# huawei-noah/Speech-Backbones

Measured on NVIDIA H100. Metric: mel-frames/sec at N=50 reverse-diffusion steps, higher is better.
Workload: dtype f32

## Files before the change

include/sbk.h:

```cpp
#ifndef SBK_H_
#define SBK_H_

#include <stddef.h>
#include <stdint.h>

#ifdef __cplusplus
extern "C" {
#endif

typedef struct sbk_handle sbk_handle;

enum { SBK_OK = 0, SBK_ERR_ARG = 1, SBK_ERR_CUDA = 2, SBK_ERR_STATE = 3, SBK_ERR_UNSUPPORTED = 4 };

enum { SBK_PREC_FP32 = 0,
       SBK_PREC_TF32 = 1,
       SBK_PREC_BF16 = 2,
       SBK_PREC_FP32X3 = 3 };

enum { SBK_MODEL_GRADTTS = 0, SBK_MODEL_DIFFVC = 1 };

typedef struct sbk_config {
    int32_t model;
    int32_t n_feats;
    int32_t dim;
// ... 9 lines not shown
    int32_t use_ref_t;
} sbk_config;

int sbk_create(const sbk_config* cfg, sbk_handle** out);
void sbk_destroy(sbk_handle* h);

int sbk_set_weight(sbk_handle* h, const char* ref_name, const void* data, const int64_t* shape, int ndim);
int sbk_pack(sbk_handle* h);
int sbk_num_weights(const sbk_handle* h);
const char* sbk_weight_name(const sbk_handle* h, int i);

size_t sbk_workspace_bytes(const sbk_handle* h, int B, int T);
size_t sbk_workspace_bytes_n(const sbk_handle* h, int B, int T, int n_timesteps);

int sbk_estimator(sbk_handle* h, const float* x, const float* mask, const float* mu, const float* t,
                  const float* spk, float* out, int B, int T, void* stream);

int sbk_reverse_diffusion(sbk_handle* h, const float* z, const float* mask, const float* mu, const float* spk,
                          const float* noise, float* out, int B, int T, int n_timesteps, int stoc, void* stream);

int sbk_vc_estimator(sbk_handle* h, const float* x, const float* mask, const float* mean, const float* cond,
                     const float* t, float* out, int B, int T, void* stream);

int sbk_vc_reverse_diffusion(sbk_handle* h, const float* z, const float* mask, const float* mean, const float* cond,
                             const float* noise, float* out, int B, int T, int n_timesteps, int mode, void* stream);

int sbk_vc_conditioning(sbk_handle* h, const float* ref, const float* ref_mask, const float* mean_ref, const float* c,
                        float* cond_out, int B, int Tr, int n_timesteps, void* stream);
int sbk_vc_cond_debug_num(const sbk_handle* h);
const char* sbk_vc_cond_debug_name(const sbk_handle* h, int i);
int sbk_vc_cond_debug_op_layout(const sbk_handle* h, const char* name);
int sbk_vc_cond_debug_read(sbk_handle* h, const char* name, void* dst, int64_t* numel);

int sbk_reverse_steps(sbk_handle* h, float* xt, const float* mask, const float* mu, const float* spk,
                      const float* noise, int B, int T, int n_timesteps, int step_begin, int step_end,
                      int stoc, void* stream);

int sbk_reverse_diffusion_host(sbk_handle* h, const float* z, const float* mask, const float* mu, const float* spk,
                               const float* noise, float* out, int B, int T, int n_timesteps, int stoc);

int sbk_prior_expand(const float* mu_x, const float* w_ceil, const float* x_mask, const int64_t* y_lengths,
                     const float* noise_tf, float temperature, int B, int F, int Tx, int Ty,
                     float* mu_y, float* z, float* y_mask, float* attn, void* stream);

int64_t sbk_last_launch_count(const sbk_handle* h);
int sbk_last_host_launches(const sbk_handle* h);

int sbk_profile_ops(sbk_handle* h, float* ms, double* flops, double* bytes, int cap, int* n_ops);

int sbk_debug_read(sbk_handle* h, const char* name, float* dst, int64_t* numel);
int sbk_debug_capture(sbk_handle* h, int on);
int sbk_debug_layout(const sbk_handle* h);
int sbk_debug_op_layout(const sbk_handle* h, const char* name);
int sbk_debug_num(const sbk_handle* h);
const char* sbk_debug_name(const sbk_handle* h, int i);

typedef struct sbk_vocoder sbk_vocoder;
typedef struct sbk_vocoder_config {
    int32_t device;
    int32_t num_mels;
    int32_t upsample_initial_channel;
    int32_t n_ups;
    int32_t upsample_rates[4];
    int32_t upsample_kernel_sizes[4];
    int32_t n_kernels;
    int32_t resblock_kernel_sizes[3];
    int32_t resblock_dilations[3][3];
} sbk_vocoder_config;
int sbk_vocoder_create(const sbk_vocoder_config* cfg, sbk_vocoder** out);
typedef struct sbk_vocoder_config_ex {
    int32_t device;
    int32_t num_mels;
    int32_t upsample_initial_channel;
    int32_t n_ups;
    int32_t upsample_rates[4];
    int32_t upsample_kernel_sizes[4];
    int32_t n_kernels;
    int32_t resblock_kernel_sizes[3];
    int32_t resblock_dilations[3][3];
    int32_t resblock;
} sbk_vocoder_config_ex;
int sbk_vocoder_create_ex(const sbk_vocoder_config_ex* cfg, sbk_vocoder** out);
void sbk_vocoder_destroy(sbk_vocoder* v);
int sbk_vocoder_num_weights(const sbk_vocoder* v);
const char* sbk_vocoder_weight_name(const sbk_vocoder* v, int i);
int sbk_vocoder_set_weight(sbk_vocoder* v, const char* name, const void* data, const int64_t* shape, int ndim);
int sbk_vocoder_pack(sbk_vocoder* v);
int sbk_vocoder_set_precision(sbk_vocoder* v, int32_t precision);
size_t sbk_vocoder_workspace_bytes(const sbk_vocoder* v, int B, int T);
int sbk_vocoder_forward(sbk_vocoder* v, const float* mel, float* wav, int B, int T, void* stream);
int64_t sbk_vocoder_last_launch_count(const sbk_vocoder* v);
int sbk_vocoder_debug_capture(sbk_vocoder* v, int on);
int sbk_vocoder_debug_num(const sbk_vocoder* v);
const char* sbk_vocoder_debug_name(const sbk_vocoder* v, int i);
int sbk_vocoder_debug_read(sbk_vocoder* v, const char* name, float* dst, int64_t* numel);
int sbk_vocoder_debug_op_layout(const sbk_vocoder* v, const char* name);

typedef struct sbk_textenc sbk_textenc;
typedef struct sbk_textenc_config {
    int32_t device;
    int32_t n_vocab, n_feats, n_channels, filter_channels, filter_channels_dp, n_heads, n_layers, kernel_size, window_size;
    int32_t n_spks, spk_emb_dim;
    int32_t kind;
} sbk_textenc_config;
int sbk_textenc_create(const sbk_textenc_config* cfg, sbk_textenc** out);
void sbk_textenc_destroy(sbk_textenc* e);
// ... 34 lines not shown
```

speech-backbones_b200/csrc/sbk_api.cu:

```cuda
#include "sbk_host.h"

#include <math.h>
#include <stdarg.h>
#include <stdio.h>
#include <stdlib.h>
#include <string.h>

#include <algorithm>
#include <map>
#include <string>
#include <vector>

using namespace sbk;

static thread_local char g_err[1024] = "";
int sbk::fail(int code, const char* fmt, ...) {
    va_list ap;
    va_start(ap, fmt);
    vsnprintf(g_err, sizeof(g_err), fmt, ap);
    va_end(ap);
    return code;
}

namespace {
// ... 1194 lines not shown
        vp.out = cond_out + (size_t)i * B * dc; vp.B = B; vp.dc = dc; vp.use_ref = cf.use_ref_t ? 1 : 0;
        n += launch_vc_cond(vp, s);
    }
    if (const cudaError_t e = h->vc_snaps.finish()) return fail(SBK_ERR_CUDA, "sbk_vc_conditioning: debug capture failed: %s", cudaGetErrorString(e));
    CU(cudaGetLastError());
    h->last_launches = n;
    return SBK_OK;
}

extern "C" int sbk_vc_cond_debug_num(const sbk_handle* h) { return h ? (int)h->vc_snaps.list.size() : 0; }
extern "C" const char* sbk_vc_cond_debug_name(const sbk_handle* h, int i) {
    if (!h || i < 0 || i >= (int)h->vc_snaps.list.size()) return nullptr;
    return h->vc_snaps.list[i].name.c_str();
}
extern "C" int sbk_vc_cond_debug_op_layout(const sbk_handle* h, const char* name) {
    const Snapshots::Snap* sn = h && name ? h->vc_snaps.find(name) : nullptr;
    return sn ? sn->fmt : -1;
}
extern "C" int sbk_vc_cond_debug_read(sbk_handle* h, const char* name, void* dst, int64_t* numel) {
    if (!h || !name) return fail(SBK_ERR_ARG, "sbk_vc_cond_debug_read: null argument");
    return h->vc_snaps.read(name, dst, numel, h->cfg.device, "sbk_vc_cond_debug_read");
}

extern "C" int sbk_prior_expand(const float* mu_x, const float* w_ceil, const float* x_mask, const int64_t* y_lengths,
                                const float* noise_tf, float temperature, int B, int F, int Tx, int Ty,
                                float* mu_y, float* z, float* y_mask, float* attn, void* stream) {
    if (!mu_x || !w_ceil || !x_mask || !y_lengths || !mu_y || !z || !y_mask) return fail(SBK_ERR_ARG, "sbk_prior_expand: null argument");
    if (B <= 0 || F <= 0 || Tx <= 0 || Ty <= 0) return fail(SBK_ERR_ARG, "sbk_prior_expand: bad sizes B=%d F=%d Tx=%d Ty=%d", B, F, Tx, Ty);
    if (Tx > 12000) return fail(SBK_ERR_ARG, "sbk_prior_expand: Tx=%d exceeds the 12000-token shared-memory table", Tx);
    if (noise_tf && !(temperature > 0.f)) return fail(SBK_ERR_ARG, "sbk_prior_expand: temperature must be > 0");
    PriorExpandParams p;
    p.mu_x = mu_x; p.w_ceil = w_ceil; p.x_mask = x_mask; p.y_len = reinterpret_cast<const long long*>(y_lengths);
    p.noise_tf = noise_tf; p.temperature = temperature; p.B = B; p.F = F; p.Tx = Tx; p.Ty = Ty;
    p.mu_y = mu_y; p.z = z; p.y_mask = y_mask; p.attn = attn;
    launch_prior_expand(p, (cudaStream_t)stream);
    CU(cudaGetLastError());
    return SBK_OK;
}

extern "C" int64_t sbk_last_launch_count(const sbk_handle* h) { return h ? h->last_launches : 0; }
extern "C" int sbk_last_host_launches(const sbk_handle* h) { return h ? h->last_host_launches : 0; }

extern "C" int sbk_debug_capture(sbk_handle* h, int on) {
    if (!h) return fail(SBK_ERR_ARG, "sbk_debug_capture: null handle");
    h->capture = h->vc_snaps.on = on != 0;
    return SBK_OK;
}
extern "C" int sbk_debug_layout(const sbk_handle* h) { return (h && h->cfg.precision != SBK_PREC_FP32) ? 1 : 0; }
extern "C" int sbk_debug_op_layout(const sbk_handle* h, const char* name) {
    if (!h || !name) return -1;
    for (auto& op : h->plan.ops) if (op.name == name) return op.dbg_fmt;
    return -1;
}
extern "C" int sbk_debug_num(const sbk_handle* h) { return h ? (int)h->plan.ops.size() : 0; }
extern "C" const char* sbk_debug_name(const sbk_handle* h, int i) {
    if (!h || i < 0 || i >= (int)h->plan.ops.size()) return nullptr;
    return h->plan.ops[i].name.c_str();
}
extern "C" int sbk_debug_read(sbk_handle* h, const char* name, float* dst, int64_t* numel) {
    if (!h || !name) return fail(SBK_ERR_ARG, "sbk_debug_read: null argument");
    for (auto& op : h->plan.ops) {
        if (op.name != name) continue;
        if (numel) *numel = op.dbg_numel;
        if (dst && op.dbg_ptr && op.dbg_numel > 0) {
            CU(cudaDeviceSynchronize());
            const void* src = op.dbg_copy ? (const void*)op.dbg_copy : (const void*)op.dbg_ptr;
            return read_widened(dst, src, op.dbg_numel, op.dbg_fmt);
        }
        return SBK_OK;
    }
    return fail(SBK_ERR_ARG, "sbk_debug_read: no intermediate named '%s'", name);
}
```

speech-backbones_b200/csrc/sbk_attn_x3.cu:

```cuda
#include "sbk_tc.cuh"

#include <type_traits>

namespace sbk {

using namespace tc;

namespace kx3 {
constexpr int PX = 64;
constexpr int KCH = 8;
constexpr int XS = KCH * PX * 16;
constexpr int WS = 2 * KCH * 128 * 16;
constexpr int STAGE = XS + WS;
constexpr int STAGES = 2;
constexpr int OPI = (PX / 4) * 128 * 16;
constexpr int THREADS = 256 + 32;
constexpr int NBARS = 2 * STAGES;
constexpr size_t SMEM = (size_t)STAGES * STAGE + 4 * OPI + 4 * 128 * 4 + NBARS * 8 + 16;
static_assert(SMEM <= 227 * 1024, "shared memory budget");
static_assert(XS <= OPI && STAGES == 2, "fp32x3: the converted x fits a context image; a K stage is the whole ring");
}

template <int MODE>
__global__ void __launch_bounds__(kx3::THREADS, 1) k_attn_kv_wg(const ConvTcParams p) {
    using namespace kx3;
    constexpr bool X3 = MODE == 2;
    constexpr int EPC = MODE == 1 ? 8 : 4;
    constexpr int KMAIN = MODE == 1 ? K_BF16 : K_TF32;
    extern __shared__ __align__(1024) uint8_t smem[];
    uint8_t* sS = smem;
    uint8_t* kp = sS + STAGES * STAGE;
    uint8_t* vt = kp + OPI;
    uint8_t* pc = vt + OPI;
    uint8_t* vc = pc + OPI;
    float* s_mx = reinterpret_cast<float*>(vc + OPI);
    float* s_z = s_mx + 2 * 128;
    uint64_t* bars = reinterpret_cast<uint64_t*>(s_z + 2 * 128);

    const int tid = threadIdx.x, warp = __shfl_sync(0xffffffffu, tid >> 5, 0), lane = tid & 31;
    const int HW = p.H * p.W;
    const int ksteps = p.c0 / (KCH * EPC);
    const int ksteps_t = X3 ? 2 * ksteps : ksteps;
    const int items = (HW + PX - 1) / PX;
    const int total = p.B * items;
    const uint32_t bar0 = smem_u32(bars);
    auto full = [&](int s) { return bar0 + 8u * s; };
    auto empty = [&](int s) { return bar0 + 8u * (STAGES + s); };

    if (tid == 0) {
        for (int s = 0; s < STAGES; ++s) { mbar_init(full(s), 1); mbar_init(empty(s), 8); }
        fence_barrier_init();
    }
    __syncthreads();

    if (warp < 8) {
        const int wg = warp >> 2, wt = tid & 127;
        const int row = tid & 127, half = tid >> 7;
        constexpr uint32_t D_HI = desc_hi(128);
        const uint32_t s0 = smem_u32(sS);
        uint32_t it = 0;
        for (int t = blockIdx.x; t < total; t += gridDim.x) {
            const int b = t / items, mt = t - b * items;
            float acc[64];
            if constexpr (X3) {
                for (int kb = 0; kb < ksteps; ++kb, it += 2) {
                    const int sc = it % STAGES, sm = (it + 1) % STAGES;
                    mbar_wait(full(sc), (it / STAGES) & 1);
                    mbar_wait(full(sm), ((it + 1) / STAGES) & 1);
                    const uint32_t xc = s0 + sc * STAGE, xm = s0 + sm * STAGE;
                    uint8_t* cx = (kb & 1) ? vc : pc;
                    {
                        const float4* src = reinterpret_cast<const float4*>(sS + sm * STAGE);
#pragma unroll
                        for (int i = tid; i < XS / 16; i += 256) {
                            const float4 v = src[i];
                            reinterpret_cast<float4*>(cx)[i] = corr_chunk(v.x, v.y, v.z, v.w);
                        }
                    }
                    fence_proxy_async();
                    asm volatile("bar.sync 1, 256;" ::: "memory");
                    const uint32_t c_lo = desc_lo(smem_u32(cx), PX * 16), x_lo = desc_lo(xm, PX * 16);
                    const uint32_t wc_lo = desc_lo(xc + XS + wg * (KCH * 128 * 16), 128 * 16), wm_lo = desc_lo(xm + XS + wg * (KCH * 128 * 16), 128 * 16);
                    wg_fence();
#pragma unroll
                    for (int kk = 0; kk < KCH / 2; ++kk)
                        wgmma<128, K_F16>(acc, desc_pack(c_lo + (uint32_t)(kk * 2 * PX), D_HI), desc_pack(wc_lo + (uint32_t)(kk * 2 * 128), D_HI),
                                          (kb | kk) != 0 ? 1u : 0u);
#pragma unroll
                    for (int kk = 0; kk < KCH / 2; ++kk)
                        wgmma<128, K_TF32>(acc, desc_pack(x_lo + (uint32_t)(kk * 2 * PX), D_HI), desc_pack(wm_lo + (uint32_t)(kk * 2 * 128), D_HI), 1u);
                    wg_commit();
                    wg_wait<0>();
                    wg_fence_regs(acc);
                    __syncwarp();
                    if (lane == 0) { mbar_arrive(empty(sc)); mbar_arrive(empty(sm)); }
                }
            } else
            for (int ks = 0; ks < ksteps_t; ++ks, ++it) {
                const int s = it % STAGES;
                mbar_wait(full(s), (it / STAGES) & 1);
                const uint32_t xs = s0 + s * STAGE;
                const uint32_t x_lo = desc_lo(xs, PX * 16), w_lo = desc_lo(xs + XS + wg * (KCH * 128 * 16), 128 * 16);
                auto issue = [&](auto kind) {
#pragma unroll
                    for (int kk = 0; kk < KCH / 2; ++kk)
                        wgmma<128, decltype(kind)::value>(acc, desc_pack(x_lo + (uint32_t)(kk * 2 * PX), D_HI),
                                                          desc_pack(w_lo + (uint32_t)(kk * 2 * 128), D_HI), (ks | kk) != 0 ? 1u : 0u);
                };
                wg_fence();
                issue(std::integral_constant<int, KMAIN>{});
                wg_commit();
                wg_wait<0>();
                wg_fence_regs(acc);
                __syncwarp();
                if (lane == 0) mbar_arrive(empty(s));
            }
            {
                uint8_t* img = wg == 0 ? kp : vt;
#pragma unroll
                for (int i = 0; i < 64; ++i) {
                    const int px = frag_row(wt, i), r = frag_col(wt, i);
                    *reinterpret_cast<float*>(img + ((size_t)(px / 4) * 128 + r) * 16 + (px % 4) * 4) = acc[i];
                }
            }
            asm volatile("bar.sync 1, 256;" ::: "memory");
            const int nvalid = min(PX, HW - mt * PX) - half * (PX / 2);
            float kr[PX / 2];
#pragma unroll
            for (int c = 0; c < PX / 8; ++c) {
                const float4 q = *reinterpret_cast<const float4*>(kp + ((size_t)(half * (PX / 8) + c) * 128 + row) * 16);
                kr[4 * c] = q.x; kr[4 * c + 1] = q.y; kr[4 * c + 2] = q.z; kr[4 * c + 3] = q.w;
            }
            float mx = -INFINITY;
#pragma unroll
            for (int i = 0; i < PX / 2; ++i) mx = fmaxf(mx, i < nvalid ? kr[i] : -INFINITY);
            s_mx[half * 128 + row] = mx;
            asm volatile("bar.sync 1, 256;" ::: "memory");
            const float md = fmaxf(s_mx[row], s_mx[128 + row]);
            float z0 = 0.f, z1 = 0.f;
#pragma unroll
            for (int i = 0; i < PX / 2; i += 2) {
                const float e0 = i < nvalid ? (X3 ? expf(kr[i] - md) : __expf(kr[i] - md)) : 0.f;
                const float e1 = i + 1 < nvalid ? (X3 ? expf(kr[i + 1] - md) : __expf(kr[i + 1] - md)) : 0.f;
                z0 += e0; z1 += e1;
                kr[i] = e0; kr[i + 1] = e1;
            }
            s_z[half * 128 + row] = z0 + z1;
#pragma unroll
            for (int c = 0; c < PX / 8; ++c) {
                const size_t o = ((size_t)(half * (PX / 8) + c) * 128 + row) * 16;
                const float e0 = kr[4 * c], e1 = kr[4 * c + 1], e2 = kr[4 * c + 2], e3 = kr[4 * c + 3];
                *reinterpret_cast<float4*>(kp + o) = make_float4(e0, e1, e2, e3);
                if constexpr (X3) {
                    *reinterpret_cast<uint4*>(pc + o) =
                        make_uint4(f16x2_sat(tf32_lo(e0) * 256.f, tf32_lo(e1) * 256.f), f16x2_sat(tf32_lo(e2) * 256.f, tf32_lo(e3) * 256.f),
                                   f16x2_sat(e0 * 0.0625f, e1 * 0.0625f), f16x2_sat(e2 * 0.0625f, e3 * 0.0625f));
                    const float4 v = *reinterpret_cast<const float4*>(vt + o);
                    *reinterpret_cast<uint4*>(vc + o) =
                        make_uint4(f16x2_sat(v.x * 0.00390625f, v.y * 0.00390625f), f16x2_sat(v.z * 0.00390625f, v.w * 0.00390625f),
                                   f16x2_sat(tf32_lo(v.x) * 16.f, tf32_lo(v.y) * 16.f), f16x2_sat(tf32_lo(v.z) * 16.f, tf32_lo(v.w) * 16.f));
                }
            }
            fence_proxy_async();
            asm volatile("bar.sync 1, 256;" ::: "memory");
            float sacc[32];
            {
                const uint32_t p_lo = desc_lo(smem_u32(kp) + 64 * wg * 16, 128 * 16), v_lo = desc_lo(smem_u32(vt) + 64 * wg * 16, 128 * 16);
                const uint32_t pc_lo = desc_lo(smem_u32(pc) + 64 * wg * 16, 128 * 16), vc_lo = desc_lo(smem_u32(vc) + 64 * wg * 16, 128 * 16);
                wg_fence();
                if constexpr (X3) {
#pragma unroll
                    for (int kk = 0; kk < PX / 8; ++kk)
                        wgmma<64, K_F16>(sacc, desc_pack(pc_lo + (uint32_t)(kk * 2 * 128), D_HI), desc_pack(vc_lo + (uint32_t)(kk * 2 * 128), D_HI),
                                         kk != 0 ? 1u : 0u);
                }
#pragma unroll
                for (int kk = 0; kk < PX / 8; ++kk)
                    wgmma<64, K_TF32>(sacc, desc_pack(p_lo + (uint32_t)(kk * 2 * 128), D_HI), desc_pack(v_lo + (uint32_t)(kk * 2 * 128), D_HI),
                                      (X3 || kk != 0) ? 1u : 0u);
                wg_commit();
                wg_wait<0>();
                wg_fence_regs(sacc);
            }
            float* pt0 = p.kv_part + ((long long)b * items + mt) * kHeads * kKvPartFloats;
            if (half == 0) {
                float* pt = pt0 + (row / 32) * kKvPartFloats;
                pt[row % 32] = md;
                pt[32 + row % 32] = s_z[row] + s_z[128 + row];
            }
#pragma unroll
            for (int i = 0; i < 32; ++i) {
                const int dl = frag_row(wt, i), el = frag_col(wt, i);
                if ((dl >> 5) == (el >> 5)) {
                    float* pt = pt0 + (2 * wg + (dl >> 5)) * kKvPartFloats;
                    pt[64 + (dl & 31) * 32 + (el & 31)] = sacc[i];
                }
            }
            asm volatile("bar.sync 1, 256;" ::: "memory");
        }
    } else {
        uint32_t it = 0;
        const int chs = p.c0 / EPC;
        for (int t = blockIdx.x; t < total; t += gridDim.x) {
            const int b = t / items, mt = t - b * items;
            const int m0 = mt * PX, m_hi = m0 + PX < HW ? m0 + PX : HW;
            const int hh0 = m0 / p.W, ww0 = m0 - hh0 * p.W;
            for (int ks = 0; ks < ksteps_t; ++ks, ++it) {
                const int s = it % STAGES;
                const int kb = X3 ? ks >> 1 : ks;
                const bool corr = X3 && (ks & 1) == 0;
                const uint32_t xs = smem_u32(sS) + s * STAGE;
                if (lane == 0) {
                    mbar_wait(empty(s), ((it / STAGES) & 1) ^ 1);
                    mbar_arrive_expect_tx(full(s), corr ? WS : STAGE);
                    bulk_g2s(xs + XS, reinterpret_cast<const uint8_t*>(p.wpk) + (size_t)(X3 ? 2 * kb + (corr ? 1 : 0) : ks) * WS, WS, full(s));
                }
                __syncwarp();
                if (lane < KCH && !corr) {
                    const uint8_t* src = reinterpret_cast<const uint8_t*>(p.in0);
                    const int k = lane, cl = kb * KCH + k;
                    int m = m0, hh = hh0, ww = ww0, qx = 0;
                    while (m < m_hi) {
                        const int n = (p.W - ww) < (m_hi - m) ? (p.W - ww) : (m_hi - m);
                        bulk_g2s(xs + (k * PX + qx) * 16, src + (((long long)(b * p.H + hh) * chs + cl) * p.W + ww) * 16,
                                 (uint32_t)n * 16u, full(s));
                        m += n; qx += n; ++hh; ww = 0;
                    }
                    if (qx < PX) bulk_g2s(xs + (k * PX + qx) * 16, p.zero_page, (uint32_t)(PX - qx) * 16u, full(s));
                }
            }
        }
    }
}

template <int MODE>
static int launch_kv(const ConvTcParams& p, cudaStream_t s) {
    static DevCache cache;
    const int num_sms = cache.get(reinterpret_cast<const void*>(k_attn_kv_wg<MODE>));
    if (num_sms <= 0) return -1;
    if (p.c0 % (kx3::KCH * (MODE == 1 ? 8 : 4)) != 0) return -1;
    const long long total = (long long)p.B * ((p.H * p.W + kx3::PX - 1) / kx3::PX);
    const int grid = (int)(total < num_sms ? total : num_sms);
    k_attn_kv_wg<MODE><<<grid, kx3::THREADS, kx3::SMEM, s>>>(p);
    return 1;
}

int attn_kv_tile_pixels() { return kx3::PX; }
int launch_attn_kv(const ConvTcParams& p, cudaStream_t s) {
    return p.form == FORM_X3 ? launch_kv<2>(p, s) : p.form == FORM_BF16 ? launch_kv<1>(p, s) : launch_kv<0>(p, s);
}

}
```

speech-backbones_b200/csrc/sbk_conv_tc.cu:

```cuda
#include "sbk_tc.cuh"

#include <cuda_fp16.h>
#include <string.h>
#include <type_traits>

namespace sbk {

namespace tc {

constexpr int TPX = 128;
constexpr int NCONS = 256;
constexpr int NTHREADS = NCONS + 128;
constexpr int NCONV = 96;
constexpr int PROD_REGS = 40, CONS_REGS = 232;
static_assert(128 * PROD_REGS + NCONS * CONS_REGS <= 65536, "register file");

template <int GEOM, int R = 1> struct Geo;
template <int R> struct Geo<G_C3, R> {
    static_assert(R == 1 || R == 2, "3x3 tiles are 1 or 2 rows");
    static constexpr int ROWS = R, HR = R + 2, PXP = TPX + 2, TAPS = 9, KCH = 2, NACC = R;
};
template <> struct Geo<G_PW> { static constexpr int ROWS = 1, HR = 1, PXP = TPX, TAPS = 1, KCH = 8, NACC = 1; };
template <> struct Geo<G_DOWN> { static constexpr int ROWS = 1, HR = 3, PXP = 2 * (TPX + 1), TAPS = 9, KCH = 2, NACC = 1; };
template <> struct Geo<G_UP> { static constexpr int ROWS = 1, HR = 3, PXP = TPX + 2, TAPS = 16, KCH = 2, NACC = 4; };
// ... 734 lines not shown
        case tc_key(G_C7, T, 64):                   return launch_tc<G_C7, T, 64>(p, s);
        case tc_key(G_C7, X, 64):                   return launch_tc<G_C7, X, 64>(p, s);
        default:                                    return -1;
    }
}

static uint32_t f32_to_tf32_rna(float x) {
    uint32_t u; memcpy(&u, &x, 4);
    if ((u & 0x7F800000u) != 0x7F800000u) u += 0x1000u;
    return u & 0xFFFFE000u;
}
static uint16_t f32_to_f16_rn(float x) {
    if (x > 65504.f) x = 65504.f;
    if (x < -65504.f) x = -65504.f;
    const __half h = __float2half_rn(x);
    uint16_t u; memcpy(&u, &h, 2);
    return u;
}
static uint16_t f32_to_bf16_rn(float x) {
    uint32_t u; memcpy(&u, &x, 4);
    if ((u & 0x7FFFFFFFu) > 0x7F800000u) return (uint16_t)((u >> 16) | 0x40);
    u += 0x7FFFu + ((u >> 16) & 1u);
    return (uint16_t)(u >> 16);
}
static void wimg_put(uint8_t* img, const ConvTcWImg& g, int co, int ks, int tap, int ch, int e, float w) {
    const size_t i = conv_tc_wimg_index(g, co, ks, tap, ch, e);
    if (g.form == FORM_BF16) {
        reinterpret_cast<uint16_t*>(img)[i] = f32_to_bf16_rn(w);
        return;
    }
    const uint32_t uh = f32_to_tf32_rna(w);
    reinterpret_cast<uint32_t*>(img)[i] = uh;
    if (g.form == FORM_X3) {
        float fh; memcpy(&fh, &uh, 4);
        uint16_t* cc = reinterpret_cast<uint16_t*>(img) + 2 * conv_tc_wimg_index(g, co, ks, tap, ch, 0, 1);
        cc[e] = f32_to_f16_rn(w);
        cc[4 + e] = f32_to_f16_rn((w - fh) * 4096.f);
    }
}

size_t conv_tc_pack_image(const float* w, int cout, int cin, int geom, int form, int nt, uint8_t* dst) {
    const ConvTcWImg g = conv_tc_wimg(geom, form, nt, cin);
    const int taps = conv_tc_taps(geom), rows = conv_tc_stage_rows(geom), epc = form_epc(form), cps = g.kch * epc;
    if (dst)
        for (int co = 0; co < cout / nt * nt; ++co) for (int ks = 0; ks < g.ksteps; ++ks) for (int tap = 0; tap < g.taps; ++tap)
            for (int ch = 0; ch < g.kch; ++ch) for (int e = 0; e < epc; ++e) {
                const int ci = ks / rows * cps + ch * epc + e;
                wimg_put(dst, g, co, ks, tap, ch, e, w[((size_t)co * cin + ci) * taps + ks % rows * g.taps + tap]);
            }
    return conv_tc_wimg_bytes(g, cout);
}

size_t attn_kv_pack_image(const float* q, int C, int form, uint8_t* dst) {
    ConvTcWImg g = conv_tc_wimg(G_PW, form, 128, C);
    g.taps = 2;
    const int epc = form_epc(form), cps = g.kch * epc;
    if (dst)
        for (int row = 0; row < 128; ++row) for (int ks = 0; ks < g.ksteps; ++ks) for (int kv = 0; kv < 2; ++kv)
            for (int ch = 0; ch < g.kch; ++ch) for (int e = 0; e < epc; ++e)
                wimg_put(dst, g, row, ks, kv, ch, e, q[(size_t)(128 + kv * 128 + row) * C + ks * cps + ch * epc + e]);
    return conv_tc_wimg_bytes(g, 128);
}

}
```

speech-backbones_b200/csrc/sbk_internal.h:

```cpp
#pragma once
#include <cuda_runtime.h>
#include <stdint.h>

namespace sbk {

constexpr int kGroups = 8;
constexpr int kHeads = 4;
constexpr int kDimHead = 32;
constexpr int kAttnHidden = 128;
constexpr int kKvPartFloats = 32 + 32 + 32 * 32;

enum Geom { G_PW = 0, G_C3 = 1, G_DOWN = 2, G_UP = 3, G_C1K3 = 4, G_C1K7 = 5, G_C1K11 = 6, G_C7 = 7, G_C1K5 = 8,
            G_C1K3W = 9, G_C1K5W = 10, G_C1K7W = 11, G_C1K11W = 12 };
__host__ __device__ constexpr bool geom_c1_wide(int g) { return g >= G_C1K3W && g <= G_C1K11W; }
__host__ __device__ constexpr bool geom_is_c1(int g) { return (g >= G_C1K3 && g <= G_C1K11) || g == G_C1K5 || geom_c1_wide(g); }
__host__ __device__ constexpr int conv_tc_c1_halo(int g) { return geom_c1_wide(g) ? 128 : 64; }
enum Pro { PRO_NONE = 0, PRO_MASK = 1, PRO_GN = 2 };
enum Epi { EPI_PLAIN = 0, EPI_RES = 1, EPI_KV = 2 };

struct GnRef {
    const double* stats;
    const float* gamma;
    const float* beta;
    float inv_count;
// ... 158 lines not shown
};
int launch_cond_fold(const CondFoldParams& p, cudaStream_t s);

struct DiffMeanParams {
    const float* ref; const float* mean_ref; const float* mask; float* out; float g; int B, H, T;
};
struct ChanStatsParams {
    const float* x; double* stats; int B, H, W, C;
};
struct InGluParams {
    const float* raw; const double* stats; const float* gamma; const float* beta;
    const float* tb;
    const float* mask; int T;
    float* out; int B, H, W, C;
    int form;
};
struct VcCondParams {
    const double* ysum;
    const float* mask; int Tr; int H;
    const float* wf; const float* bf;
    const float* c;
    const float* freqs; float t; int dim;
    const float* w0; const float* b0; const float* w2; const float* b2;
    float* out;
    int B, dc, use_ref;
};
int launch_diff_mean(const DiffMeanParams& p, cudaStream_t s);
int launch_chan_stats(const ChanStatsParams& p, cudaStream_t s);
int launch_in_glu(const InGluParams& p, cudaStream_t s);
int launch_vc_cond(const VcCondParams& p, cudaStream_t s);

struct PriorExpandParams {
    const float* mu_x;
    const float* w_ceil;
    const float* x_mask;
    const long long* y_len;
    const float* noise_tf;
    float temperature;
    int B, F, Tx, Ty;
    float* mu_y; float* z;
    float* y_mask;
    float* attn;
};
int launch_prior_expand(const PriorExpandParams& p, cudaStream_t s);

struct StepBeginParams { double* stats; int n_doubles; int* step_cur; int* step_next; };

int launch_igemm(const IgemmParams& p, cudaStream_t s);
int launch_first_conv(const FirstConvParams& p, cudaStream_t s);
int launch_conv_tc(const ConvTcParams& p, cudaStream_t s);
int conv_tc_ntile(int geom, int Cout, int form);
size_t conv_tc_pack_image(const float* w, int cout, int cin, int geom, int form, int nt, uint8_t* dst);
size_t attn_kv_pack_image(const float* qkv, int C, int form, uint8_t* dst);
int launch_gn_act(const GnActParams& p, cudaStream_t s);
int launch_resfinal(const ResFinalParams& p, cudaStream_t s);
int launch_attn_ctx(const AttnCtxParams& p, cudaStream_t s);
int attn_kv_tile_pixels();
int launch_attn_kv(const ConvTcParams& p, cudaStream_t s);
int launch_attn_mix(const AttnMixParams& p, cudaStream_t s);
int launch_final(const FinalParams& p, cudaStream_t s);
int launch_time_table(const TimeTableParams& p, cudaStream_t s);
int launch_spk(const SpkParams& p, cudaStream_t s);
int launch_step_begin(const StepBeginParams& p, cudaStream_t s);
int device_sm_count();
int launch_scale_mask(const float* z, const float* mask, float* out, long long n_per_b_row, int B, int H, int T, cudaStream_t s);

__device__ __forceinline__ float tf32_lo(float x) { return x - __uint_as_float(__float_as_uint(x) & 0xFFFFE000u); }

constexpr float kCorrDown = 1.f / 4096.f;
constexpr float kCorrUp = 4096.f;
__device__ __forceinline__ uint32_t f16x2_sat(float e0, float e1) {
    uint32_t d;
    asm("cvt.rn.satfinite.f16x2.f32 %0, %1, %2;" : "=r"(d) : "f"(e1), "f"(e0));
    return d;
}
__device__ __forceinline__ float4 corr_chunk(float x0, float x1, float x2, float x3) {
    return make_float4(__uint_as_float(f16x2_sat(tf32_lo(x0), tf32_lo(x1))), __uint_as_float(f16x2_sat(tf32_lo(x2), tf32_lo(x3))),
                       __uint_as_float(f16x2_sat(x0 * kCorrDown, x1 * kCorrDown)), __uint_as_float(f16x2_sat(x2 * kCorrDown, x3 * kCorrDown)));
}

inline int igemm_mtiles(int geom, int Hout, int Wout, int Hin, int Win) {
    const int TM = 128;
    if (geom == G_UP) return 4 * ((Hin * Win + TM - 1) / TM);
    return (Hout * Wout + TM - 1) / TM;
}

}
```

Baseline: 14250.

## Pair pixel tiles per weight stage in attention KV kernel and deepen pipeline

The attention key/value projection kernel can now process two pixel tiles per block. They share each staged weight chunk, so weight traffic is amortised, and a heuristic enables pairing only when it shortens the per-SM wave count. The pipeline gets three stages for tf32/bf16, warp-specialised register reallocation via setmaxnreg, and a single producer warp. For fp32x3, weights are now packed raw and split into tf32 plus an f16 correction on device each stage, instead of prepacking both parts. This adds per-step conversion work and register pressure from two accumulators.

```diff
diff --git a/include/sbk.h b/include/sbk.h
--- a/include/sbk.h
+++ b/include/sbk.h
@@ -85,6 +85,8 @@
 int sbk_debug_capture(sbk_handle* h, int on);
 int sbk_debug_layout(const sbk_handle* h);
 int sbk_debug_op_layout(const sbk_handle* h, const char* name);
+size_t sbk_debug_attn_kv_image(const float* qkv, int C, int precision, void* dst);
+int sbk_debug_attn_kv_tiles(int B, int items, int num_sms, int* tiles);
 int sbk_debug_num(const sbk_handle* h);
 const char* sbk_debug_name(const sbk_handle* h, int i);
 
diff --git a/speech-backbones_b200/csrc/sbk_api.cu b/speech-backbones_b200/csrc/sbk_api.cu
--- a/speech-backbones_b200/csrc/sbk_api.cu
+++ b/speech-backbones_b200/csrc/sbk_api.cu
@@ -1270,6 +1270,22 @@
     for (auto& op : h->plan.ops) if (op.name == name) return op.dbg_fmt;
     return -1;
 }
+extern "C" size_t sbk_debug_attn_kv_image(const float* qkv, int C, int precision, void* dst) {
+    const int form = precision == SBK_PREC_TF32 ? FORM_TF32 : precision == SBK_PREC_BF16 ? FORM_BF16
+                   : precision == SBK_PREC_FP32X3 ? FORM_X3 : -1;
+    if (!qkv || C <= 0 || C % 64 != 0 || form < 0) return 0;
+    return attn_kv_pack_image(qkv, C, form, reinterpret_cast<uint8_t*>(dst));
+}
+extern "C" int sbk_debug_attn_kv_tiles(int B, int items, int num_sms, int* tiles) {
+    if (B <= 0 || items <= 0 || num_sms <= 0) return 0;
+    const int pair = attn_kv_pairs(B, items, num_sms), n = attn_kv_tiles(B, items, pair);
+    if (tiles)
+        for (int t = 0; t < n; ++t) {
+            const AttnKvTile k = attn_kv_tile(t, items, pair);
+            tiles[3 * t] = k.b; tiles[3 * t + 1] = k.item; tiles[3 * t + 2] = k.n;
+        }
+    return n;
+}
 extern "C" int sbk_debug_num(const sbk_handle* h) { return h ? (int)h->plan.ops.size() : 0; }
 extern "C" const char* sbk_debug_name(const sbk_handle* h, int i) {
     if (!h || i < 0 || i >= (int)h->plan.ops.size()) return nullptr;
diff --git a/speech-backbones_b200/csrc/sbk_attn_x3.cu b/speech-backbones_b200/csrc/sbk_attn_x3.cu
--- a/speech-backbones_b200/csrc/sbk_attn_x3.cu
+++ b/speech-backbones_b200/csrc/sbk_attn_x3.cu
@@ -11,20 +11,24 @@
 constexpr int KCH = 8;
 constexpr int XS = KCH * PX * 16;
 constexpr int WS = 2 * KCH * 128 * 16;
-constexpr int STAGE = XS + WS;
-constexpr int STAGES = 2;
+constexpr int STAGE = 2 * XS + WS;
 constexpr int OPI = (PX / 4) * 128 * 16;
-constexpr int THREADS = 256 + 32;
-constexpr int NBARS = 2 * STAGES;
-constexpr size_t SMEM = (size_t)STAGES * STAGE + 4 * OPI + 4 * 128 * 4 + NBARS * 8 + 16;
-static_assert(SMEM <= 227 * 1024, "shared memory budget");
-static_assert(XS <= OPI && STAGES == 2, "fp32x3: the converted x fits a context image; a K stage is the whole ring");
+constexpr int THREADS = 256 + 128;
+constexpr int PROD_REGS = 40, CONS_REGS = 232;
+static_assert(128 * PROD_REGS + 256 * CONS_REGS <= 65536, "register file");
+__host__ __device__ constexpr int stages(int mode) { return mode == 2 ? 2 : 3; }
+__host__ __device__ constexpr size_t smem(int mode) {
+    return (size_t)stages(mode) * STAGE + (mode == 2 ? 4 : 2) * OPI + 4 * 128 * 4 + 2 * stages(mode) * 8;
+}
+static_assert(smem(0) <= 227 * 1024 && smem(1) <= 227 * 1024 && smem(2) <= 227 * 1024, "shared memory budget");
+static_assert(2 * XS <= OPI && WS <= OPI, "fp32x3: the converted stage fits Pc (activations) and Vc (weights)");
 }
 
 template <int MODE>
-__global__ void __launch_bounds__(kx3::THREADS, 1) k_attn_kv_wg(const ConvTcParams p) {
+__global__ void __launch_bounds__(kx3::THREADS, 1) k_attn_kv_wg(const ConvTcParams p, int pair) {
     using namespace kx3;
     constexpr bool X3 = MODE == 2;
+    constexpr int STAGES = stages(MODE);
     constexpr int EPC = MODE == 1 ? 8 : 4;
     constexpr int KMAIN = MODE == 1 ? K_BF16 : K_TF32;
     extern __shared__ __align__(1024) uint8_t smem[];
@@ -33,16 +37,15 @@
     uint8_t* vt = kp + OPI;
     uint8_t* pc = vt + OPI;
     uint8_t* vc = pc + OPI;
-    float* s_mx = reinterpret_cast<float*>(vc + OPI);
+    float* s_mx = reinterpret_cast<float*>(X3 ? vc + OPI : pc);
     float* s_z = s_mx + 2 * 128;
     uint64_t* bars = reinterpret_cast<uint64_t*>(s_z + 2 * 128);
 
     const int tid = threadIdx.x, warp = __shfl_sync(0xffffffffu, tid >> 5, 0), lane = tid & 31;
     const int HW = p.H * p.W;
     const int ksteps = p.c0 / (KCH * EPC);
-    const int ksteps_t = X3 ? 2 * ksteps : ksteps;
     const int items = (HW + PX - 1) / PX;
-    const int total = p.B * items;
+    const int total = attn_kv_tiles(p.B, items, pair);
     const uint32_t bar0 = smem_u32(bars);
     auto full = [&](int s) { return bar0 + 8u * s; };
     auto empty = [&](int s) { return bar0 + 8u * (STAGES + s); };
@@ -54,179 +57,188 @@
     __syncthreads();
 
     if (warp < 8) {
+        setmaxnreg_inc<CONS_REGS>();
         const int wg = warp >> 2, wt = tid & 127;
         const int row = tid & 127, half = tid >> 7;
         constexpr uint32_t D_HI = desc_hi(128);
         const uint32_t s0 = smem_u32(sS);
         uint32_t it = 0;
         for (int t = blockIdx.x; t < total; t += gridDim.x) {
-            const int b = t / items, mt = t - b * items;
-            float acc[64];
-            if constexpr (X3) {
-                for (int kb = 0; kb < ksteps; ++kb, it += 2) {
-                    const int sc = it % STAGES, sm = (it + 1) % STAGES;
-                    mbar_wait(full(sc), (it / STAGES) & 1);
-                    mbar_wait(full(sm), ((it + 1) / STAGES) & 1);
-                    const uint32_t xc = s0 + sc * STAGE, xm = s0 + sm * STAGE;
-                    uint8_t* cx = (kb & 1) ? vc : pc;
-                    {
-                        const float4* src = reinterpret_cast<const float4*>(sS + sm * STAGE);
-#pragma unroll
-                        for (int i = tid; i < XS / 16; i += 256) {
-                            const float4 v = src[i];
-                            reinterpret_cast<float4*>(cx)[i] = corr_chunk(v.x, v.y, v.z, v.w);
-                        }
-                    }
-                    fence_proxy_async();
-                    asm volatile("bar.sync 1, 256;" ::: "memory");
-                    const uint32_t c_lo = desc_lo(smem_u32(cx), PX * 16), x_lo = desc_lo(xm, PX * 16);
-                    const uint32_t wc_lo = desc_lo(xc + XS + wg * (KCH * 128 * 16), 128 * 16), wm_lo = desc_lo(xm + XS + wg * (KCH * 128 * 16), 128 * 16);
-                    wg_fence();
-#pragma unroll
-                    for (int kk = 0; kk < KCH / 2; ++kk)
-                        wgmma<128, K_F16>(acc, desc_pack(c_lo + (uint32_t)(kk * 2 * PX), D_HI), desc_pack(wc_lo + (uint32_t)(kk * 2 * 128), D_HI),
-                                          (kb | kk) != 0 ? 1u : 0u);
-#pragma unroll
-                    for (int kk = 0; kk < KCH / 2; ++kk)
-                        wgmma<128, K_TF32>(acc, desc_pack(x_lo + (uint32_t)(kk * 2 * PX), D_HI), desc_pack(wm_lo + (uint32_t)(kk * 2 * 128), D_HI), 1u);
-                    wg_commit();
-                    wg_wait<0>();
-                    wg_fence_regs(acc);
-                    __syncwarp();
-                    if (lane == 0) { mbar_arrive(empty(sc)); mbar_arrive(empty(sm)); }
-                }
-            } else
-            for (int ks = 0; ks < ksteps_t; ++ks, ++it) {
+            const AttnKvTile tile = attn_kv_tile(t, items, pair);
+            float acc0[64], acc1[64];
+            for (int ks = 0; ks < ksteps; ++ks, ++it) {
                 const int s = it % STAGES;
                 mbar_wait(full(s), (it / STAGES) & 1);
                 const uint32_t xs = s0 + s * STAGE;
-                const uint32_t x_lo = desc_lo(xs, PX * 16), w_lo = desc_lo(xs + XS + wg * (KCH * 128 * 16), 128 * 16);
-                auto issue = [&](auto kind) {
+                const uint32_t w_lo = desc_lo(xs + 2 * XS + wg * (KCH * 128 * 16), 128 * 16);
+                if constexpr (X3) {
+                    if (ks) asm volatile("bar.sync 1, 256;" ::: "memory");
+                    uint8_t* st = sS + s * STAGE;
+#pragma unroll
+                    for (int i = tid; i < WS / 16; i += 256) {
+                        float4* wp = reinterpret_cast<float4*>(st + 2 * XS) + i;
+                        const float4 w = *wp;
+                        uint32_t h0, h1, h2, h3;
+                        asm("cvt.rna.tf32.f32 %0, %1;" : "=r"(h0) : "f"(w.x));
+                        asm("cvt.rna.tf32.f32 %0, %1;" : "=r"(h1) : "f"(w.y));
+                        asm("cvt.rna.tf32.f32 %0, %1;" : "=r"(h2) : "f"(w.z));
+                        asm("cvt.rna.tf32.f32 %0, %1;" : "=r"(h3) : "f"(w.w));
+                        *wp = make_float4(__uint_as_float(h0), __uint_as_float(h1), __uint_as_float(h2), __uint_as_float(h3));
+                        reinterpret_cast<uint4*>(vc)[i] = make_uint4(
+                            f16x2_sat(w.x, w.y), f16x2_sat(w.z, w.w),
+                            f16x2_sat((w.x - __uint_as_float(h0)) * kCorrUp, (w.y - __uint_as_float(h1)) * kCorrUp),
+                            f16x2_sat((w.z - __uint_as_float(h2)) * kCorrUp, (w.w - __uint_as_float(h3)) * kCorrUp));
+                    }
+#pragma unroll
+                    for (int i = tid; i < 2 * XS / 16; i += 256) {
+                        const float4 v = reinterpret_cast<const float4*>(st)[i];
+                        reinterpret_cast<float4*>(pc)[i] = corr_chunk(v.x, v.y, v.z, v.w);
+                    }
+                    fence_proxy_async();
+                    asm volatile("bar.sync 1, 256;" ::: "memory");
+                }
+                auto issue = [&](float (&acc)[64], int j) {
+                    const uint32_t x_lo = desc_lo(xs + j * XS, PX * 16);
+                    if constexpr (X3) {
+                        const uint32_t c_lo = desc_lo(smem_u32(pc) + j * XS, PX * 16), wc_lo = desc_lo(smem_u32(vc) + wg * (KCH * 128 * 16), 128 * 16);
+#pragma unroll
+                        for (int kk = 0; kk < KCH / 2; ++kk)
+                            wgmma<128, K_F16>(acc, desc_pack(c_lo + (uint32_t)(kk * 2 * PX), D_HI), desc_pack(wc_lo + (uint32_t)(kk * 2 * 128), D_HI),
+                                              (ks | kk) != 0 ? 1u : 0u);
+                    }
 #pragma unroll
                     for (int kk = 0; kk < KCH / 2; ++kk)
-                        wgmma<128, decltype(kind)::value>(acc, desc_pack(x_lo + (uint32_t)(kk * 2 * PX), D_HI),
-                                                          desc_pack(w_lo + (uint32_t)(kk * 2 * 128), D_HI), (ks | kk) != 0 ? 1u : 0u);
+                        wgmma<128, KMAIN>(acc, desc_pack(x_lo + (uint32_t)(kk * 2 * PX), D_HI), desc_pack(w_lo + (uint32_t)(kk * 2 * 128), D_HI),
+                                          (X3 || (ks | kk) != 0) ? 1u : 0u);
                 };
                 wg_fence();
-                issue(std::integral_constant<int, KMAIN>{});
+                issue(acc0, 0);
+                issue(acc1, 1);
                 wg_commit();
                 wg_wait<0>();
-                wg_fence_regs(acc);
+                wg_fence_regs(acc0);
+                wg_fence_regs(acc1);
                 __syncwarp();
                 if (lane == 0) mbar_arrive(empty(s));
             }
-            {
-                uint8_t* img = wg == 0 ? kp : vt;
-#pragma unroll
-                for (int i = 0; i < 64; ++i) {
-                    const int px = frag_row(wt, i), r = frag_col(wt, i);
-                    *reinterpret_cast<float*>(img + ((size_t)(px / 4) * 128 + r) * 16 + (px % 4) * 4) = acc[i];
-                }
-            }
-            asm volatile("bar.sync 1, 256;" ::: "memory");
-            const int nvalid = min(PX, HW - mt * PX) - half * (PX / 2);
-            float kr[PX / 2];
-#pragma unroll
-            for (int c = 0; c < PX / 8; ++c) {
-                const float4 q = *reinterpret_cast<const float4*>(kp + ((size_t)(half * (PX / 8) + c) * 128 + row) * 16);
-                kr[4 * c] = q.x; kr[4 * c + 1] = q.y; kr[4 * c + 2] = q.z; kr[4 * c + 3] = q.w;
-            }
-            float mx = -INFINITY;
-#pragma unroll
-            for (int i = 0; i < PX / 2; ++i) mx = fmaxf(mx, i < nvalid ? kr[i] : -INFINITY);
-            s_mx[half * 128 + row] = mx;
-            asm volatile("bar.sync 1, 256;" ::: "memory");
-            const float md = fmaxf(s_mx[row], s_mx[128 + row]);
-            float z0 = 0.f, z1 = 0.f;
-#pragma unroll
-            for (int i = 0; i < PX / 2; i += 2) {
-                const float e0 = i < nvalid ? (X3 ? expf(kr[i] - md) : __expf(kr[i] - md)) : 0.f;
-                const float e1 = i + 1 < nvalid ? (X3 ? expf(kr[i + 1] - md) : __expf(kr[i + 1] - md)) : 0.f;
-                z0 += e0; z1 += e1;
-                kr[i] = e0; kr[i + 1] = e1;
-            }
-            s_z[half * 128 + row] = z0 + z1;
-#pragma unroll
-            for (int c = 0; c < PX / 8; ++c) {
-                const size_t o = ((size_t)(half * (PX / 8) + c) * 128 + row) * 16;
-                const float e0 = kr[4 * c], e1 = kr[4 * c + 1], e2 = kr[4 * c + 2], e3 = kr[4 * c + 3];
-                *reinterpret_cast<float4*>(kp + o) = make_float4(e0, e1, e2, e3);
-                if constexpr (X3) {
-                    *reinterpret_cast<uint4*>(pc + o) =
-                        make_uint4(f16x2_sat(tf32_lo(e0) * 256.f, tf32_lo(e1) * 256.f), f16x2_sat(tf32_lo(e2) * 256.f, tf32_lo(e3) * 256.f),
-                                   f16x2_sat(e0 * 0.0625f, e1 * 0.0625f), f16x2_sat(e2 * 0.0625f, e3 * 0.0625f));
-                    const float4 v = *reinterpret_cast<const float4*>(vt + o);
-                    *reinterpret_cast<uint4*>(vc + o) =
-                        make_uint4(f16x2_sat(v.x * 0.00390625f, v.y * 0.00390625f), f16x2_sat(v.z * 0.00390625f, v.w * 0.00390625f),
-                                   f16x2_sat(tf32_lo(v.x) * 16.f, tf32_lo(v.y) * 16.f), f16x2_sat(tf32_lo(v.z) * 16.f, tf32_lo(v.w) * 16.f));
-                }
-            }
-            fence_proxy_async();
-            asm volatile("bar.sync 1, 256;" ::: "memory");
-            float sacc[32];
-            {
-                const uint32_t p_lo = desc_lo(smem_u32(kp) + 64 * wg * 16, 128 * 16), v_lo = desc_lo(smem_u32(vt) + 64 * wg * 16, 128 * 16);
-                const uint32_t pc_lo = desc_lo(smem_u32(pc) + 64 * wg * 16, 128 * 16), vc_lo = desc_lo(smem_u32(vc) + 64 * wg * 16, 128 * 16);
-                wg_fence();
-                if constexpr (X3) {
+            auto context = [&](float (&acc)[64], int mt) {
+                {
+                    uint8_t* img = wg == 0 ? kp : vt;
+#pragma unroll
+                    for (int i = 0; i < 64; ++i) {
+                        const int px = frag_row(wt, i), r = frag_col(wt, i);
+                        *reinterpret_cast<float*>(img + ((size_t)(px / 4) * 128 + r) * 16 + (px % 4) * 4) = acc[i];
+                    }
+                }
+                asm volatile("bar.sync 1, 256;" ::: "memory");
+                const int nvalid = min(PX, HW - mt * PX) - half * (PX / 2);
+                float kr[PX / 2];
+#pragma unroll
+                for (int c = 0; c < PX / 8; ++c) {
+                    const float4 q = *reinterpret_cast<const float4*>(kp + ((size_t)(half * (PX / 8) + c) * 128 + row) * 16);
+                    kr[4 * c] = q.x; kr[4 * c + 1] = q.y; kr[4 * c + 2] = q.z; kr[4 * c + 3] = q.w;
+                }
+                float mx = -INFINITY;
+#pragma unroll
+                for (int i = 0; i < PX / 2; ++i) mx = fmaxf(mx, i < nvalid ? kr[i] : -INFINITY);
+                s_mx[half * 128 + row] = mx;
+                asm volatile("bar.sync 1, 256;" ::: "memory");
+                const float md = fmaxf(s_mx[row], s_mx[128 + row]);
+                float z0 = 0.f, z1 = 0.f;
+#pragma unroll
+                for (int i = 0; i < PX / 2; i += 2) {
+                    const float e0 = i < nvalid ? (X3 ? expf(kr[i] - md) : __expf(kr[i] - md)) : 0.f;
+                    const float e1 = i + 1 < nvalid ? (X3 ? expf(kr[i + 1] - md) : __expf(kr[i + 1] - md)) : 0.f;
+                    z0 += e0; z1 += e1;
+                    kr[i] = e0; kr[i + 1] = e1;
+                }
+                s_z[half * 128 + row] = z0 + z1;
+#pragma unroll
+                for (int c = 0; c < PX / 8; ++c) {
+                    const size_t o = ((size_t)(half * (PX / 8) + c) * 128 + row) * 16;
+                    const float e0 = kr[4 * c], e1 = kr[4 * c + 1], e2 = kr[4 * c + 2], e3 = kr[4 * c + 3];
+                    *reinterpret_cast<float4*>(kp + o) = make_float4(e0, e1, e2, e3);
+                    if constexpr (X3) {
+                        *reinterpret_cast<uint4*>(pc + o) =
+                            make_uint4(f16x2_sat(tf32_lo(e0) * 256.f, tf32_lo(e1) * 256.f), f16x2_sat(tf32_lo(e2) * 256.f, tf32_lo(e3) * 256.f),
+                                       f16x2_sat(e0 * 0.0625f, e1 * 0.0625f), f16x2_sat(e2 * 0.0625f, e3 * 0.0625f));
+                        const float4 v = *reinterpret_cast<const float4*>(vt + o);
+                        *reinterpret_cast<uint4*>(vc + o) =
+                            make_uint4(f16x2_sat(v.x * 0.00390625f, v.y * 0.00390625f), f16x2_sat(v.z * 0.00390625f, v.w * 0.00390625f),
+                                       f16x2_sat(tf32_lo(v.x) * 16.f, tf32_lo(v.y) * 16.f), f16x2_sat(tf32_lo(v.z) * 16.f, tf32_lo(v.w) * 16.f));
+                    }
+                }
+                fence_proxy_async();
+                asm volatile("bar.sync 1, 256;" ::: "memory");
+                float sacc[32];
+                {
+                    const uint32_t p_lo = desc_lo(smem_u32(kp) + 64 * wg * 16, 128 * 16), v_lo = desc_lo(smem_u32(vt) + 64 * wg * 16, 128 * 16);
+                    const uint32_t pc_lo = desc_lo(smem_u32(pc) + 64 * wg * 16, 128 * 16), vc_lo = desc_lo(smem_u32(vc) + 64 * wg * 16, 128 * 16);
+                    wg_fence();
+                    if constexpr (X3) {
+#pragma unroll
+                        for (int kk = 0; kk < PX / 8; ++kk)
+                            wgmma<64, K_F16>(sacc, desc_pack(pc_lo + (uint32_t)(kk * 2 * 128), D_HI), desc_pack(vc_lo + (uint32_t)(kk * 2 * 128), D_HI),
+                                             kk != 0 ? 1u : 0u);
+                    }
 #pragma unroll
                     for (int kk = 0; kk < PX / 8; ++kk)
-                        wgmma<64, K_F16>(sacc, desc_pack(pc_lo + (uint32_t)(kk * 2 * 128), D_HI), desc_pack(vc_lo + (uint32_t)(kk * 2 * 128), D_HI),
-                                         kk != 0 ? 1u : 0u);
-                }
-#pragma unroll
-                for (int kk = 0; kk < PX / 8; ++kk)
-                    wgmma<64, K_TF32>(sacc, desc_pack(p_lo + (uint32_t)(kk * 2 * 128), D_HI), desc_pack(v_lo + (uint32_t)(kk * 2 * 128), D_HI),
-                                      (X3 || kk != 0) ? 1u : 0u);
-                wg_commit();
-                wg_wait<0>();
-                wg_fence_regs(sacc);
-            }
-            float* pt0 = p.kv_part + ((long long)b * items + mt) * kHeads * kKvPartFloats;
-            if (half == 0) {
-                float* pt = pt0 + (row / 32) * kKvPartFloats;
-                pt[row % 32] = md;
-                pt[32 + row % 32] = s_z[row] + s_z[128 + row];
-            }
-#pragma unroll
-            for (int i = 0; i < 32; ++i) {
-                const int dl = frag_row(wt, i), el = frag_col(wt, i);
-                if ((dl >> 5) == (el >> 5)) {
-                    float* pt = pt0 + (2 * wg + (dl >> 5)) * kKvPartFloats;
-                    pt[64 + (dl & 31) * 32 + (el & 31)] = sacc[i];
-                }
-            }
-            asm volatile("bar.sync 1, 256;" ::: "memory");
+                        wgmma<64, K_TF32>(sacc, desc_pack(p_lo + (uint32_t)(kk * 2 * 128), D_HI), desc_pack(v_lo + (uint32_t)(kk * 2 * 128), D_HI),
+                                          (X3 || kk != 0) ? 1u : 0u);
+                    wg_commit();
+                    wg_wait<0>();
+                    wg_fence_regs(sacc);
+                }
+                float* pt0 = p.kv_part + ((long long)tile.b * items + mt) * kHeads * kKvPartFloats;
+                if (half == 0) {
+                    float* pt = pt0 + (row / 32) * kKvPartFloats;
+                    pt[row % 32] = md;
+                    pt[32 + row % 32] = s_z[row] + s_z[128 + row];
+                }
+#pragma unroll
+                for (int i = 0; i < 32; ++i) {
+                    const int dl = frag_row(wt, i), el = frag_col(wt, i);
+                    if ((dl >> 5) == (el >> 5)) {
+                        float* pt = pt0 + (2 * wg + (dl >> 5)) * kKvPartFloats;
+                        pt[64 + (dl & 31) * 32 + (el & 31)] = sacc[i];
+                    }
+                }
+                asm volatile("bar.sync 1, 256;" ::: "memory");
+            };
+            context(acc0, tile.item);
+            if (tile.n == 2) context(acc1, tile.item + 1);
         }
     } else {
+        setmaxnreg_dec<PROD_REGS>();
+        if (warp != 8) return;
         uint32_t it = 0;
         const int chs = p.c0 / EPC;
         for (int t = blockIdx.x; t < total; t += gridDim.x) {
-            const int b = t / items, mt = t - b * items;
-            const int m0 = mt * PX, m_hi = m0 + PX < HW ? m0 + PX : HW;
+            const AttnKvTile tile = attn_kv_tile(t, items, pair);
+            const int j = lane >> 3, k = lane & 7;
+            const int m0 = (tile.item + j) * PX, m_hi = j < tile.n ? min(m0 + PX, HW) : m0;
             const int hh0 = m0 / p.W, ww0 = m0 - hh0 * p.W;
-            for (int ks = 0; ks < ksteps_t; ++ks, ++it) {
+            for (int ks = 0; ks < ksteps; ++ks, ++it) {
                 const int s = it % STAGES;
-                const int kb = X3 ? ks >> 1 : ks;
-                const bool corr = X3 && (ks & 1) == 0;
                 const uint32_t xs = smem_u32(sS) + s * STAGE;
                 if (lane == 0) {
                     mbar_wait(empty(s), ((it / STAGES) & 1) ^ 1);
-                    mbar_arrive_expect_tx(full(s), corr ? WS : STAGE);
-                    bulk_g2s(xs + XS, reinterpret_cast<const uint8_t*>(p.wpk) + (size_t)(X3 ? 2 * kb + (corr ? 1 : 0) : ks) * WS, WS, full(s));
+                    mbar_arrive_expect_tx(full(s), STAGE);
+                    bulk_g2s(xs + 2 * XS, reinterpret_cast<const uint8_t*>(p.wpk) + (size_t)ks * WS, WS, full(s));
                 }
                 __syncwarp();
-                if (lane < KCH && !corr) {
+                if (lane < 2 * KCH) {
                     const uint8_t* src = reinterpret_cast<const uint8_t*>(p.in0);
-                    const int k = lane, cl = kb * KCH + k;
+                    const int cl = ks * KCH + k;
+                    const uint32_t xj = xs + j * XS + k * PX * 16;
                     int m = m0, hh = hh0, ww = ww0, qx = 0;
                     while (m < m_hi) {
                         const int n = (p.W - ww) < (m_hi - m) ? (p.W - ww) : (m_hi - m);
-                        bulk_g2s(xs + (k * PX + qx) * 16, src + (((long long)(b * p.H + hh) * chs + cl) * p.W + ww) * 16,
+                        bulk_g2s(xj + qx * 16, src + (((long long)(tile.b * p.H + hh) * chs + cl) * p.W + ww) * 16,
                                  (uint32_t)n * 16u, full(s));
                         m += n; qx += n; ++hh; ww = 0;
                     }
-                    if (qx < PX) bulk_g2s(xs + (k * PX + qx) * 16, p.zero_page, (uint32_t)(PX - qx) * 16u, full(s));
+                    if (qx < PX) bulk_g2s(xj + qx * 16, p.zero_page, (uint32_t)(PX - qx) * 16u, full(s));
                 }
             }
         }
@@ -239,9 +251,10 @@
     const int num_sms = cache.get(reinterpret_cast<const void*>(k_attn_kv_wg<MODE>));
     if (num_sms <= 0) return -1;
     if (p.c0 % (kx3::KCH * (MODE == 1 ? 8 : 4)) != 0) return -1;
-    const long long total = (long long)p.B * ((p.H * p.W + kx3::PX - 1) / kx3::PX);
+    const int items = (p.H * p.W + kx3::PX - 1) / kx3::PX, pair = attn_kv_pairs(p.B, items, num_sms);
+    const long long total = attn_kv_tiles(p.B, items, pair);
     const int grid = (int)(total < num_sms ? total : num_sms);
-    k_attn_kv_wg<MODE><<<grid, kx3::THREADS, kx3::SMEM, s>>>(p);
+    k_attn_kv_wg<MODE><<<grid, kx3::THREADS, kx3::smem(MODE), s>>>(p, pair);
     return 1;
 }
 
diff --git a/speech-backbones_b200/csrc/sbk_conv_tc.cu b/speech-backbones_b200/csrc/sbk_conv_tc.cu
--- a/speech-backbones_b200/csrc/sbk_conv_tc.cu
+++ b/speech-backbones_b200/csrc/sbk_conv_tc.cu
@@ -810,13 +810,17 @@
 }
 
 size_t attn_kv_pack_image(const float* q, int C, int form, uint8_t* dst) {
-    ConvTcWImg g = conv_tc_wimg(G_PW, form, 128, C);
+    const bool raw = form == FORM_X3;
+    ConvTcWImg g = conv_tc_wimg(G_PW, raw ? FORM_TF32 : form, 128, C);
     g.taps = 2;
-    const int epc = form_epc(form), cps = g.kch * epc;
+    const int epc = form_epc(g.form), cps = g.kch * epc;
     if (dst)
         for (int row = 0; row < 128; ++row) for (int ks = 0; ks < g.ksteps; ++ks) for (int kv = 0; kv < 2; ++kv)
-            for (int ch = 0; ch < g.kch; ++ch) for (int e = 0; e < epc; ++e)
-                wimg_put(dst, g, row, ks, kv, ch, e, q[(size_t)(128 + kv * 128 + row) * C + ks * cps + ch * epc + e]);
+            for (int ch = 0; ch < g.kch; ++ch) for (int e = 0; e < epc; ++e) {
+                const float w = q[(size_t)(128 + kv * 128 + row) * C + ks * cps + ch * epc + e];
+                if (raw) reinterpret_cast<float*>(dst)[conv_tc_wimg_index(g, row, ks, kv, ch, e)] = w;
+                else wimg_put(dst, g, row, ks, kv, ch, e, w);
+            }
     return conv_tc_wimg_bytes(g, 128);
 }
 
diff --git a/speech-backbones_b200/csrc/sbk_internal.h b/speech-backbones_b200/csrc/sbk_internal.h
--- a/speech-backbones_b200/csrc/sbk_internal.h
+++ b/speech-backbones_b200/csrc/sbk_internal.h
@@ -234,6 +234,16 @@
 int conv_tc_ntile(int geom, int Cout, int form);
 size_t conv_tc_pack_image(const float* w, int cout, int cin, int geom, int form, int nt, uint8_t* dst);
 size_t attn_kv_pack_image(const float* qkv, int C, int form, uint8_t* dst);
+struct AttnKvTile { int b, item, n; };
+__host__ __device__ inline int attn_kv_tiles(int B, int items, int pair) { return B * (pair ? (items + 1) / 2 : items); }
+__host__ __device__ inline AttnKvTile attn_kv_tile(int t, int items, int pair) {
+    const int per = pair ? (items + 1) / 2 : items, b = t / per, item = (pair ? 2 : 1) * (t - b * per);
+    return {b, item, pair && items - item >= 2 ? 2 : 1};
+}
+__host__ __device__ inline int attn_kv_pairs(int B, int items, int num_sms) {
+    const int w1 = (attn_kv_tiles(B, items, 0) + num_sms - 1) / num_sms, w2 = (attn_kv_tiles(B, items, 1) + num_sms - 1) / num_sms;
+    return 7 * w2 <= 4 * w1 ? 1 : 0;
+}
 int launch_gn_act(const GnActParams& p, cudaStream_t s);
 int launch_resfinal(const ResFinalParams& p, cudaStream_t s);
 int launch_attn_ctx(const AttnCtxParams& p, cudaStream_t s);
```

Result: faster. 14420 (median of 6 runs) (+1.2%).
